# jameshensman/pyvb

Hardware: AMD Instinct MI355X
Metric: VB update iterations/sec (T=10k, D=64, N=1024 LDS); ELBO rel-err vs NumPy (higher is better)
Workload: dtype f64; 1 GPU; LDS T=10000 D=64 K=64, 1024 replicates per GPU (BASELINE configs[2]); replicates_total=1024, parallelism=replicates sharded over 1 GPU(s), collective=none (1 GPU), degraded=False

## Files before the change

### pyvb_amd/csrc/api.hip

```cpp
#include "common.h"
#include <cstdarg>
#include <cstdio>
#include <cstdlib>
#include <cstring>
#include <cmath>
#include <vector>
#include <mutex>
#include <dlfcn.h>

static thread_local char g_err[512] = "";

void pyvb_set_error(const char* fmt, ...) {
    va_list ap; va_start(ap, fmt);
    vsnprintf(g_err, sizeof(g_err), fmt, ap);
    va_end(ap);
}

int pyvb_hip_fail(hipError_t e, const char* what, const char* file, int line) {
    pyvb_set_error("HIP error %d (%s) in %s at %s:%d", (int)e, hipGetErrorString(e), what, file, line);
    return PYVB_E_HIP;
}

TimedLaunch::TimedLaunch(pyvb_lds* h_, int k_, hipStream_t s_) : h(h_), slot(-1), s(s_ ? s_ : h_->stream) {
    if (!h->timing) return;
// ... 80 lines not shown
    h->pool = (EventPair*)calloc(PYVB_EVENT_POOL, sizeof(EventPair));
    for (int i = 0; i < PYVB_EVENT_POOL; ++i) { TRYHIP(hipEventCreate(&h->pool[i].e0)); TRYHIP(hipEventCreate(&h->pool[i].e1)); }
    const size_t n = (size_t)N;
    TRY(dev_alloc(&h->Y, n * T * K));
    TRY(dev_alloc(&h->Syy, n * K));
    TRY(dev_alloc(&h->X[0], n * T * L.DP));
    TRY(dev_alloc(&h->X[1], n * T * L.DP));
    TRY(dev_alloc(&h->A_mean, n * D * D));
    TRY(dev_alloc(&h->A_var, n * D * D));
    TRY(dev_alloc(&h->C_mean, n * K * D));
    TRY(dev_alloc(&h->C_var, n * D * K));
    TRY(dev_alloc(&h->Q_a, n * D)); TRY(dev_alloc(&h->Q_b, n * D));
    TRY(dev_alloc(&h->R_a, n * K)); TRY(dev_alloc(&h->R_b, n * K));
    TRY(dev_alloc(&h->qld_A, n * D)); TRY(dev_alloc(&h->qld_C, n * D));
    TRY(dev_alloc(&h->Sigma, n * 3 * D * D)); TRY(dev_alloc(&h->Sigma_new, n * 3 * D * D));
    TRY(dev_alloc(&h->qld_x, n * 3)); TRY(dev_alloc(&h->qld_x_new, n * 3));
    TRY(dev_alloc(&h->lnd_A, n * D)); TRY(dev_alloc(&h->lnd_C, n * D));
    TRY(dev_alloc(&h->lnd_x, n * 3)); TRY(dev_alloc(&h->lnd_x_new, n * 3));
    TRY(dev_alloc(&h->gains, n * L.gains_total));
    TRY(dev_alloc(&h->scratch, g.scratch));
    TRY(dev_alloc(&h->zeros, 128));
    TRY(dev_alloc(&h->U, n * T * L.DP));
    TRY(h->mem.alloc((void**)&h->warm, n * 2 * sizeof(int)));
    TRY(dev_alloc(&h->stats, g.stats));
    TRY(dev_alloc(&h->mom, g.mom));
    TRY(dev_alloc(&h->sxx, g.sxx));
    if (g.U2) TRY(dev_alloc(&h->U2, g.U2));
    TRY(dev_alloc(&h->trash, g.trash));
    TRY(dev_alloc(&h->resQ, n * D)); TRY(dev_alloc(&h->resR, n * K));
    TRY(dev_alloc(&h->elbo, n * 6)); TRY(dev_alloc(&h->elbo_sum, 8));
    TRY(dev_alloc(&h->elbo_hist, (size_t)PYVB_ELBO_HISTORY * 8));
    TRY(h->mem.alloc((void**)&h->status, n * sizeof(int)));
    TRY(h->mem.alloc((void**)&h->active, n, 1));
    TRY(h->mem.alloc((void**)&h->counted, n, 1));
    TRY(h->mem.alloc((void**)&h->conv, n));
    TRY(h->mem.alloc((void**)&h->conv_iters, n * sizeof(int)));
    TRY(h->mem.alloc((void**)&h->conv_llb, n * sizeof(double), 0xFF));
    TRYHIP(hipHostMalloc((void**)&h->running_host, sizeof(double), hipHostMallocDefault));
    TRYHIP(hipEventCreateWithFlags(&h->ev_check, hipEventDisableTiming));
    if (ragged) {
        TRY(h->mem.alloc((void**)&h->len, n * sizeof(int)));
        TRYHIP(hipMemcpy(h->len, lengths, n * sizeof(int), hipMemcpyHostToDevice));
    }
    if (tied) {
        const Replicates& r = h->rep;
        TRY(h->mem.alloc((void**)&h->mstart, r.model_starts().size() * sizeof(int)));
        TRY(h->mem.alloc((void**)&h->first, n));
        TRYHIP(hipMemcpy(h->mstart, r.model_starts().data(), r.model_starts().size() * sizeof(int), hipMemcpyHostToDevice));
        TRYHIP(hipMemcpy(h->first, r.first_flags().data(), n, hipMemcpyHostToDevice));
    }
    h->status_host.assign(n, 0);
    h->reported.assign(n, 0);
    TRY(dev_alloc(&h->pri_block, g.priors));
    double* p = h->pri_block;
    h->pri.x0_mean = p; p += D; h->pri.x0_prec = p; p += D * D;
    h->pri.A_pm = p; p += D * D; h->pri.A_pp = p; p += D * D;
    h->pri.C_pm = p; p += K * D; h->pri.C_pp = p; p += D * K;
    h->pri.Q_a0 = p; p += D; h->pri.Q_b0 = p; p += D; h->pri.R_a0 = p; p += K; h->pri.R_b0 = p; p += K;
    h->pri.A_obs = p; p += D * D; h->pri.C_obs = p; p += K * D;
    h->pri.A_pld = p; p += D; h->pri.C_pld = p; p += D;
    h->pri.Q_w0 = p; p += D * D; h->pri.R_w0 = p; p += K * K;
    if (h->dense) {
        TRY(dev_alloc(&h->Q_w, n * D * D)); TRY(dev_alloc(&h->R_w, n * K * K));
        TRY(dev_alloc(&h->Qbar, n * D * D)); TRY(dev_alloc(&h->Rbar, n * K * K));
        TRY(dev_alloc(&h->lnd, n * 4));
        TRY(dev_alloc(&h->QA, n * D * D)); TRY(dev_alloc(&h->RC, n * K * D));
        TRY(dev_alloc(&h->trA, n * D)); TRY(dev_alloc(&h->trC, n * D));
        TRY(dev_alloc(&h->A_cov, n * D * cov_stride(D))); TRY(dev_alloc(&h->C_cov, n * D * cov_stride(K)));
        TRY(dev_alloc(&h->SyyF, n * K * K));
        TRY(dev_alloc(&h->RQ, n * D * D)); TRY(dev_alloc(&h->RR, n * K * K));
        TRY(dev_alloc(&h->SG, g.SG));
        TRY(dev_alloc(&h->ldm, n * 2 * D));
    }
    TRYHIP(hipMemset(h->pri.A_obs, 0xFF, ((size_t)D * D + (size_t)K * D) * sizeof(double)));
    h->st.T = T;
    h->st.fresh = (unsigned char*)calloc(T, 1);
    h->world = 1;
    {
        std::vector<double> nanv(n * (size_t)(D > 3 ? D : 3), NAN);
        TRYHIP(hipMemcpy(h->qld_x, nanv.data(), n * 3 * sizeof(double), hipMemcpyHostToDevice));
        TRYHIP(hipMemcpy(h->qld_A, nanv.data(), n * D * sizeof(double), hipMemcpyHostToDevice));
        TRYHIP(hipMemcpy(h->qld_C, nanv.data(), n * D * sizeof(double), hipMemcpyHostToDevice));
        TRYHIP(hipMemcpy(h->lnd_x, nanv.data(), n * 3 * sizeof(double), hipMemcpyHostToDevice));
        TRYHIP(hipMemcpy(h->lnd_A, nanv.data(), n * D * sizeof(double), hipMemcpyHostToDevice));
        TRYHIP(hipMemcpy(h->lnd_C, nanv.data(), n * D * sizeof(double), hipMemcpyHostToDevice));
    }
#undef dev_alloc
#undef TRY
#undef TRYHIP
    *out = h;
    return PYVB_OK;
}

int pyvb_lds_create(pyvb_lds** out, int device, int N, int T, int D, int K, int noise_kind) {
    return lds_create(out, device, N, T, D, K, noise_kind, nullptr, nullptr);
}
int pyvb_lds_create_lengths(pyvb_lds** out, int device, int N, int T, int D, int K, int noise_kind, const int* lengths) {
    return lds_create(out, device, N, T, D, K, noise_kind, lengths, nullptr);
}
int pyvb_lds_create_tied(pyvb_lds** out, int device, int N, int T, int D, int K, int noise_kind, const int* lengths, const int* model) {
    return lds_create(out, device, N, T, D, K, noise_kind, lengths, model);
}

int pyvb_lds_get_models(pyvb_lds* h, int* model) {
    ARGCHK(h, "handle is NULL");
    ARGCHK(model, "model is NULL");
// ... 32 lines not shown
    if (h->rep.n_active() == h->N) return PYVB_OK;
    int rc;
    if (h->st.x_park != h->st.cur && (rc = launch_carry(h, h->X[h->st.x_park], h->X[h->st.cur], (size_t)h->T * h->L.DP))) return rc;
    if (h->st.cls_parked_other) {
        if ((rc = launch_carry(h, h->Sigma_new, h->Sigma, (size_t)3 * h->D * h->D))) return rc;
        if ((rc = launch_carry(h, h->qld_x_new, h->qld_x, 3))) return rc;
        if ((rc = launch_carry(h, h->lnd_x_new, h->lnd_x, 3))) return rc;
    }
    h->st.parked_here();
    return PYVB_OK;
}

static int h2d(pyvb_lds* h, double* dst, const double* src, size_t n) { return to_device(h->stream, dst, src, n); }
static int d2h(pyvb_lds* h, double* dst, const double* src, size_t n) { return to_host(h->stream, dst, src, n); }

static void fill_padding(const pyvb_lds* h, double* a, size_t per, double value) {
    if (!h->rep.ragged() || !a) return;
    for (size_t n = 0; n < (size_t)h->N; ++n)
        for (size_t i = ((size_t)n * h->T + h->rep.length((int)n)) * per; i < (size_t)(n + 1) * h->T * per; ++i) a[i] = value;
}

static int host_lndet(const double* Ain, int D, double* out) {
    std::vector<double> A(Ain, Ain + (size_t)D * D);
    double s = 0.0;
    for (int j = 0; j < D; ++j) {
        double piv = A[j * D + j];
        for (int k = 0; k < j; ++k) piv -= A[j * D + k] * A[j * D + k];
        if (!(piv > 0.0)) return PYVB_E_LINALG;
        double d = sqrt(piv);
        A[j * D + j] = d; s += log(d);
        for (int i = j + 1; i < D; ++i) {
            double v = A[i * D + j];
            for (int k = 0; k < j; ++k) v -= A[i * D + k] * A[j * D + k];
            A[i * D + j] = v / d;
        }
    }
    *out = 2.0 * s;
    return PYVB_OK;
}

int pyvb_lds_set_priors(pyvb_lds* h, const double* x0_mean, const double* x0_prec,
                        const double* A_pm, const double* A_pp, const double* C_pm, const double* C_pp,
                        const double* Q_a0, const double* Q_b0, const double* R_a0, const double* R_b0) {
    ENTER(h);
    ARGCHK(x0_mean && x0_prec && A_pm && A_pp && C_pm && C_pp, "the priors of X_0 and of the columns are required");
    ARGCHK(h->dense || (Q_a0 && Q_b0 && R_a0 && R_b0), "the Gamma priors of Q and R are required");
    const int D = h->D, K = h->K, N = h->N;
    for (int i = 0; i < D * D; ++i) ARGCHK(A_pp[i] > 0.0, "A_prior_prec must be positive");
    for (int i = 0; i < D * K; ++i) ARGCHK(C_pp[i] > 0.0, "C_prior_prec must be positive");
    if (host_lndet(x0_prec, D, &h->pri.x0_lndet) != PYVB_OK) { pyvb_set_error("x0_prec is not positive definite"); return PYVB_E_LINALG; }
    int rc;
    if ((rc = h2d(h, h->pri.x0_mean, x0_mean, D))) return rc;
    if ((rc = h2d(h, h->pri.x0_prec, x0_prec, (size_t)D * D))) return rc;
    if ((rc = h2d(h, h->pri.A_pm, A_pm, (size_t)D * D))) return rc;
    if ((rc = h2d(h, h->pri.A_pp, A_pp, (size_t)D * D))) return rc;
    if ((rc = h2d(h, h->pri.C_pm, C_pm, (size_t)K * D))) return rc;
    if ((rc = h2d(h, h->pri.C_pp, C_pp, (size_t)D * K))) return rc;
    {
        std::vector<double> ld(2 * (size_t)D, 0.0);
        for (int i = 0; i < D; ++i) {
            for (int k = 0; k < D; ++k) ld[i] += log(A_pp[(size_t)i * D + k]);
            for (int k = 0; k < K; ++k) ld[D + i] += log(C_pp[(size_t)i * K + k]);
        }
        HIPCHK(hipMemcpyAsync(h->pri.A_pld, ld.data(), 2 * (size_t)D * sizeof(double), hipMemcpyHostToDevice, h->stream));
        HIPCHK(hipStreamSynchronize(h->stream));
    }
    if (!h->dense) {
        if ((rc = h2d(h, h->pri.Q_a0, Q_a0, D))) return rc;
        if ((rc = h2d(h, h->pri.Q_b0, Q_b0, D))) return rc;
        if ((rc = h2d(h, h->pri.R_a0, R_a0, K))) return rc;
        if ((rc = h2d(h, h->pri.R_b0, R_b0, K))) return rc;
        std::vector<double> qa((size_t)N * D), ra((size_t)N * K);
        std::vector<long> cq, cr;
        h->rep.children(cq, cr);
        for (int n = 0; n < N; ++n) {
            const long nq = cq[n], nr = cr[n];
            for (int k = 0; k < D; ++k)
                qa[(size_t)n * D + k] = (h->noise == PYVB_NOISE_GAMMA) ? Q_a0[0] + 0.5 * D * nq : Q_a0[k] + 0.5 * nq;
            for (int k = 0; k < K; ++k)
                ra[(size_t)n * K + k] = (h->noise == PYVB_NOISE_GAMMA) ? R_a0[0] + 0.5 * K * nr : R_a0[k] + 0.5 * nr;
        }
        if ((rc = h2d(h, h->Q_a, qa.data(), qa.size()))) return rc;
        if ((rc = h2d(h, h->R_a, ra.data(), ra.size()))) return rc;
        HIPCHK(hipStreamSynchronize(h->stream));
    }
    h->ard[0].on = h->ard[1].on = false;
    h->st.parameters_changed();
    return PYVB_OK;
}

static int ard_which(const pyvb_lds* h, int which, bool need_on) {
    ARGCHK(which == 0 || which == 1, "which must be 0 (A) or 1 (C)");
    if (need_on && !h->ard[which].on) {
        pyvb_set_error("the columns of %s have Constant precision parents: no hyperpriors were given (pyvb_lds_set_column_precisions)",
                       which == 0 ? "A" : "C");
        return PYVB_E_ARG;
    }
    return PYVB_OK;
}

int pyvb_lds_set_column_precisions(pyvb_lds* h, int which, const double* a0, const double* b0, const double* qb) {
    ARGCHK(h, "handle is NULL");
    int rc = ard_which(h, which, false);
    if (rc) return rc;
    if (h->dense) {
        pyvb_set_error("Gamma precision parents of the columns are served with DiagonalGamma and Gamma noise only, not with Wishart noise (k_wishart.hip)");
// ... 970 lines not shown
```

### pyvb_amd/csrc/common.h

```cpp
#pragma once
#include <cstdint>
#include "host.h"
#include "geometry.h"
#include "replicates.h"

struct pyvb_comm;
typedef double d4 __attribute__((ext_vector_type(4)));
typedef double d2 __attribute__((ext_vector_type(2)));

struct Priors {
    double *x0_mean, *x0_prec, *A_pm, *A_pp, *C_pm, *C_pp, *Q_a0, *Q_b0, *R_a0, *R_b0;
    double *A_obs, *C_obs;
    double *Q_w0, *R_w0;
    double *A_pld, *C_pld;
    double x0_lndet;
    double Q_a0_host, R_a0_host, Q_w0_lndet, R_w0_lndet;
};

struct ArdBuffers {
    bool on;
    double *a0, *b0, *qa;
    double *qb, *ex, *ld_ref, *ld_exact;
};

struct EventPair;
struct KernelTimer {
    double total_ms; int launches;
};

struct pyvb_lds {
    int device, N, T, D, K, noise;
    bool big;
    double* U2;
    Layout L;
    hipStream_t stream;
    struct EventPair* pool; int pool_used;
    double *Y, *Syy;
    double *X[2];
    double *A_mean, *A_var, *C_mean, *C_var;
    double *Q_a, *Q_b, *R_a, *R_b;
    double *qld_A, *qld_C;
    double *lnd_A, *lnd_C;
    int bound;
    Priors pri;
    double *pri_block;
    ArdBuffers ard[2];
    double *Sigma, *qld_x;
    double *Sigma_new, *qld_x_new;
    double *lnd_x, *lnd_x_new;
    double *gains;
    double *scratch;
    int *warm;
    double *zeros;
    double *trash;
    double *U;
    double *stats; int nchunk, chunk_len;
    int W;
    double *sxx;
    double *mom;
    double *resQ, *resR;
    double *elbo, *elbo_sum;
    int *status;
    Replicates rep;
    unsigned char *active;
    unsigned char *counted;
    unsigned char *conv;
    int *conv_iters;
    double *conv_llb;
    double *running_host;
    hipEvent_t ev_check;
    int *len;
    int *mstart;
    unsigned char *first;
    std::vector<int> status_host, reported;
    LdsState st;
    DeviceBuffers mem;
    bool timing; KernelTimer timers[PYVB_K_COUNT]; int timing_errors;
    pyvb_comm* comm; int rank, world;
    bool dense;
    double *Q_w, *R_w;
    double *Qbar, *Rbar;
    double *lnd;
    double *QA, *RC;
    double *trA, *trC;
    double *A_cov, *C_cov;
    double *SyyF;
    double *RQ, *RR;
    double *ldm;
    double *SG;
    bool has_missing;
    double *Yobs, *Yvar, *Yqld, *Yent;
    double *Ylnd, *YentX;
    double *Yld, *YcovS;
    hipStream_t side;
    hipEvent_t ev_params, ev_elbo;
    bool elbo_in_flight;
    double* elbo_hist; int hist_count;
};
#define PYVB_ELBO_HISTORY 4096

int launch_prep(pyvb_lds* h);
int launch_sweep(pyvb_lds* h, int direction, int src, bool read_cache, bool keep_x);
int launch_step(pyvb_lds* h, int t);
int launch_syy(pyvb_lds* h);
int launch_permute(pyvb_lds* h, const double* src, double* dst, int to_internal);
int launch_carry(pyvb_lds* h, const double* src, double* dst, size_t per);
int launch_stats(pyvb_lds* h, bool with_sxx);
int launch_moments(pyvb_lds* h, bool sxx_from_sweep);
int launch_observe(pyvb_lds* h);
int launch_tie(pyvb_lds* h, double* buf, size_t per);
int launch_cols(pyvb_lds* h, int which, int c0, int c1, int fuse = 0);
int launch_resid(pyvb_lds* h, int which);
int launch_ard(pyvb_lds* h, int which, bool derive);
int launch_noise(pyvb_lds* h, int which);
int launch_elbo(pyvb_lds* h, hipStream_t stream = nullptr);
int launch_elbo_sum(pyvb_lds* h, double* out = nullptr, hipStream_t stream = nullptr);
int launch_converge(pyvb_lds* h, double tol, bool first, hipStream_t stream);
int launch_prep_big(pyvb_lds* h);
int big_prepare_kernels();
int launch_sweep_big(pyvb_lds* h, int direction, int src, bool cached);
int launch_step_big(pyvb_lds* h, int t);
int launch_stats_big(pyvb_lds* h);
int launch_cols_big(pyvb_lds* h, int which, int c0, int c1, int fuse);
int launch_wexpect(pyvb_lds* h);
int launch_dense_pre(pyvb_lds* h);
int launch_cols_dense(pyvb_lds* h, int which, int c0, int c1);
int launch_wresid(pyvb_lds* h, int which, int update, bool use_sg);
int launch_syy_full(pyvb_lds* h);
int launch_elbo_dense(pyvb_lds* h, hipStream_t stream = nullptr);
int launch_colvar_to_cov(pyvb_lds* h);
int launch_cov_to_colvar(pyvb_lds* h);
int launch_cov_observe(pyvb_lds* h);
int launch_cov_convert(pyvb_lds* h, int which, double* dense, int n0, int count, int to_packed);
int launch_wexpect_big(pyvb_lds* h);
int launch_dense_pre_big(pyvb_lds* h);
int launch_cols_dense_big(pyvb_lds* h, int which, int c0, int c1);
int launch_wresid_big(pyvb_lds* h, int which, int update, bool use_sg);
int launch_syy_full_big(pyvb_lds* h);
int launch_missing_init(pyvb_lds* h, const double* Yq0, const double* Yrowvar0);
int launch_impute(pyvb_lds* h);
int launch_syy_missing(pyvb_lds* h);
int launch_impute_dense(pyvb_lds* h);
int launch_missing_ent_dense(pyvb_lds* h, int diag_cov);

struct pyvb_comm {
    void* nccl;
    pyvb_host_allreduce_fn fn; void* user;
    double* host; size_t cap;
};
int pyvb_comm_create(pyvb_comm** comm, const char id[128], int rank, int world);
int pyvb_comm_create_host(pyvb_comm** comm, pyvb_host_allreduce_fn fn, void* user);
void pyvb_comm_free(pyvb_comm* comm);
int pyvb_allreduce_f64(pyvb_comm* comm, double* buf, size_t count, hipStream_t stream);

// ... 9 lines not shown
```

### pyvb_amd/csrc/k_prep.hip

```cpp
#include "common.h"
#include "gj.h"

struct PrepArgs {
    const double *A_mean, *A_var, *C_mean, *C_var, *Q_a, *Q_b, *R_a, *R_b, *x0_mean, *x0_prec;
    double *Sigma, *qld, *lnd, *gains, *scratch;
    const double *Qbar, *QA, *RC, *trA, *trC;
    int *warm, *status;
    const unsigned char* active;
    int N, T, D, K;
    Layout L;
};

#define PREP_THREADS 256
#define MFMA(a, b, c) __builtin_amdgcn_mfma_f64_16x16x4f64((a), (b), (c), 0, 0, 0)

template <int MT, int NT, int KS, class FA, class FB, class FS>
__device__ __forceinline__ void mm(int wave, int lane, FA a_at, FB b_at, FS store) {
    const int r = lane & 15, q = lane >> 4;
    for (int m = wave; m < MT; m += 4) {
        d4 acc[NT];
#pragma unroll
        for (int n = 0; n < NT; ++n) acc[n] = d4{0, 0, 0, 0};
#pragma unroll 4
        for (int s = 0; s < KS; ++s) {
            const double av = a_at(16 * m + r, 4 * s + q);
#pragma unroll
            for (int n = 0; n < NT; ++n) acc[n] = MFMA(av, b_at(4 * s + q, 16 * n + r), acc[n]);
        }
#pragma unroll
        for (int n = 0; n < NT; ++n)
#pragma unroll
            for (int e = 0; e < 4; ++e) store(16 * m + 4 * e + q, 16 * n + r, acc[n][e]);
    }
}

template <int NT, int KS, class FA, class FB>
__device__ __forceinline__ void mm_acc(int m, int lane, FA a_at, FB b_at, d4 (&acc)[NT]) {
    const int r = lane & 15, q = lane >> 4;
#pragma unroll
    for (int n = 0; n < NT; ++n) acc[n] = d4{0, 0, 0, 0};
#pragma unroll 4
    for (int s = 0; s < KS; ++s) {
        const double av = a_at(16 * m + r, 4 * s + q);
#pragma unroll
        for (int n = 0; n < NT; ++n) acc[n] = MFMA(av, b_at(4 * s + q, 16 * n + r), acc[n]);
    }
}
template <int NT, class FS>
__device__ __forceinline__ void mm_out(int m, int lane, const d4 (&acc)[NT], FS store) {
    const int r = lane & 15, q = lane >> 4;
#pragma unroll
    for (int n = 0; n < NT; ++n)
#pragma unroll
        for (int e = 0; e < 4; ++e) store(16 * m + 4 * e + q, 16 * n + r, acc[n][e]);
}

__device__ __forceinline__ double inf_norm(const double* A, int LD, int D, int tid, double* red) {
// ... 151 lines not shown
    __syncthreads();
    gj_inverse<3>(sig, D, tid, gjbuf, gjbuf + 3 * 2 * GJ_BUF);
    if (tid < 64) {
#pragma unroll
        for (int c = 0; c < 3; ++c) {
            double lp = 0.0;
            if (tid < D) {
                const double piv = gjbuf[3 * 2 * GJ_BUF + c * 64 + tid];
                if (!(piv > 0.0)) atomicOr(a.status + n, PYVB_FAIL_STATES);
                lp = log(piv);
            }
#pragma unroll
            for (int o = 32; o > 0; o >>= 1) lp += __shfl_xor(lp, o, 64);
            if (tid == 0) { a.qld[(size_t)n * 3 + c] = 0.5 / (0.5 * lp); a.lnd[(size_t)n * 3 + c] = -lp; }
        }
    }
    if ((D & 3) == 0) {
#pragma unroll
        for (int c = 0; c < 3; ++c)
#pragma unroll
            for (int ra = 0; ra < 4; ++ra) {
                const int i = 4 * ta + ra, j0 = 4 * tb;
                if (i < D && j0 < D)
                    *reinterpret_cast<d4*>(a.Sigma + ((size_t)n * 3 + c) * D * D + (size_t)i * D + j0) = d4{sig[c][4 * ra], sig[c][4 * ra + 1], sig[c][4 * ra + 2], sig[c][4 * ra + 3]};
            }
    } else {
#pragma unroll
    for (int c = 0; c < 3; ++c)
#pragma unroll
        for (int ra = 0; ra < 4; ++ra)
#pragma unroll
            for (int cb = 0; cb < 4; ++cb) {
                const int i = 4 * ta + ra, j = 4 * tb + cb;
                if (i < D && j < D) a.Sigma[((size_t)n * 3 + c) * D * D + i * D + j] = sig[c][4 * ra + cb];
            }
    }

#pragma unroll
    for (int ra = 0; ra < 4; ++ra) {
        const int i = 4 * ta + ra, j0 = 4 * tb;
        if (i < DP && j0 < DP) {
            d4 s0, s2;
#pragma unroll
            for (int cb = 0; cb < 4; ++cb) {
                const bool in = i < D && j0 + cb < D;
                s0[cb] = in ? sig[0][4 * ra + cb] : 0.0;
                s2[cb] = in ? sig[2][4 * ra + cb] : 0.0;
            }
            *reinterpret_cast<d4*>(g + L.oS0 + (size_t)i * DP + j0) = s0;
            *reinterpret_cast<d4*>(g + L.oS2 + (size_t)i * DP + j0) = s2;
        }
    }
    if (tid < 64) { g[L.oqr + tid] = qbar[tid]; g[L.oqr + 64 + tid] = rbar[tid]; }
    if (tid < DP) {
        double s = 0.0;
        if (tid < D) for (int j = 0; j < D; ++j) s += a.x0_prec[tid * D + j] * a.x0_mean[j];
        g[L.ow0 + tid] = s;
    }
#pragma unroll
    for (int ra = 0; ra < 4; ++ra)
#pragma unroll
        for (int cb = 0; cb < 4; ++cb) {
            const int i = 4 * ta + ra, j = 4 * tb + cb;
            if (i < D && j < D) P[i * LD + j] = sig[1][4 * ra + cb];
        }
    __syncthreads();
    if constexpr (STAGE) {
        constexpr int KP = 16 * KT;
        for (int idx = tid; idx < DP * DP; idx += PREP_THREADS) W[(idx / DP) * LD + idx % DP] = qbar[idx / DP] * A_at(idx / DP, idx % DP);
        __syncthreads();
        d4 facc[DT], acc[DT], gacc[KT];
        if (wave < DT) {
            mm_acc<DT, DS>(wave, lane, [&](int i, int k) { return P[i * LD + k]; }, [&](int k, int j) { return W[k * LD + j]; }, facc);
            mm_out<DT>(wave, lane, facc, [&](int i, int j, double v) { if (i < D && j < D) g[L.oFn + pos_nat(i, j, DS)] = v; });
            mm_acc<DT, DS>(wave, lane, [&](int i, int k) { return P[i * LD + k]; }, [&](int k, int j) { return W[j * LD + k]; }, acc);
            mm_out<DT>(wave, lane, acc, [&](int i, int j, double v) { if (i < D && j < D) g[L.oBn + pos_nat(i, j, DS)] = v; });
        }
        __syncthreads();
        for (int idx = tid; idx < KP * DP; idx += PREP_THREADS) W[(idx / DP) * LD + idx % DP] = rbar[idx / DP] * C_at(idx / DP, idx % DP);
        __syncthreads();
        if (wave < DT) {
            mm_acc<KT, DS>(wave, lane, [&](int i, int k) { return P[i * LD + k]; }, [&](int k, int l) { return W[l * LD + k]; }, gacc);
            mm_out<KT>(wave, lane, gacc, [&](int i, int l, double v) { if (i < D && l < K) g[L.oGp + pos_perm(i, l, KS)] = v; });
        }
        __syncthreads();
        if (wave < DT) mm_out<DT>(wave, lane, facc, [&](int i, int j, double v) { W[i * LD + j] = (i < D && j < D) ? v : 0.0; });
    } else
    {
        mm<DT, DT, DS>(wave, lane,
                       [&](int i, int k) { return P[i * LD + k]; },
                       [&](int k, int j) { if constexpr (DENSE) return QA_at(k, j); else return qbar[k] * A_at(k, j); },
                       [&](int i, int j, double v) {
                           if (i < D && j < D) { g[L.oFn + pos_nat(i, j, DS)] = v; W[i * LD + j] = v; }
                       });
        mm<DT, DT, DS>(wave, lane,
                       [&](int i, int k) { return P[i * LD + k]; },
                       [&](int k, int j) { if constexpr (DENSE) return QA_at(j, k); else return A_at(j, k) * qbar[j]; },
                       [&](int i, int j, double v) {
                           if (i < D && j < D) g[L.oBn + pos_nat(i, j, DS)] = v;
                       });
        mm<DT, KT, DS>(wave, lane,
                       [&](int i, int k) { return P[i * LD + k]; },
                       [&](int k, int l) { if constexpr (DENSE) return RC_at(l, k); else return C_at(l, k) * rbar[l]; },
                       [&](int i, int l, double v) {
                           if (i < D && l < K) g[L.oGp + pos_perm(i, l, KS)] = v;
                       });
    }
    __syncthreads();

    int J = warmup_length<DT>(W, P, LD, D, tid, rowp);
    if (tid == 0) a.warm[n * 2 + 0] = J;
    __syncthreads();
    for (int idx = tid; idx < DP * LD; idx += PREP_THREADS) {
        const int i = idx / LD, j = idx % LD;
        W[idx] = (i < D && j < D) ? g[L.oBn + pos_nat(j, i, DS)] : 0.0;
    }
    __syncthreads();
    J = warmup_length<DT>(W, P, LD, D, tid, rowp);
    if (tid == 0) a.warm[n * 2 + 1] = J;
}

template <int DT, int KT>
static void launch_prep_t(pyvb_lds* h, const PrepArgs& a) {
    if (h->dense) hipLaunchKernelGGL((k_prep<DT, KT, true>), dim3(h->N), dim3(PREP_THREADS), 0, h->stream, a);
    else hipLaunchKernelGGL((k_prep<DT, KT, false>), dim3(h->N), dim3(PREP_THREADS), 0, h->stream, a);
}

int launch_prep(pyvb_lds* h) {
    if (h->big) return launch_prep_big(h);
    PrepArgs a;
    a.A_mean = h->A_mean; a.A_var = h->A_var; a.C_mean = h->C_mean; a.C_var = h->C_var;
    a.Q_a = h->Q_a; a.Q_b = h->Q_b; a.R_a = h->R_a; a.R_b = h->R_b;
    a.x0_mean = h->pri.x0_mean; a.x0_prec = h->pri.x0_prec;
    a.Sigma = h->Sigma_new; a.qld = h->qld_x_new; a.lnd = h->lnd_x_new; a.gains = h->gains; a.scratch = h->scratch;
    a.warm = h->warm; a.status = h->status; a.active = h->active;
    a.Qbar = h->Qbar; a.QA = h->QA; a.RC = h->RC; a.trA = h->trA; a.trC = h->trC;
    a.N = h->N; a.T = h->T; a.D = h->D; a.K = h->K; a.L = h->L;
    {
        TimedLaunch tl(h, PYVB_K_PREP);
        switch (h->L.DT * 10 + h->L.KT) {
            case 11: launch_prep_t<1, 1>(h, a); break;
            case 12: launch_prep_t<1, 2>(h, a); break;
            case 14: launch_prep_t<1, 4>(h, a); break;
            case 21: launch_prep_t<2, 1>(h, a); break;
            case 22: launch_prep_t<2, 2>(h, a); break;
            case 24: launch_prep_t<2, 4>(h, a); break;
            case 41: launch_prep_t<4, 1>(h, a); break;
            case 42: launch_prep_t<4, 2>(h, a); break;
            case 44: launch_prep_t<4, 4>(h, a); break;
            default: pyvb_set_error("unsupported tile shape"); return PYVB_E_ARG;
        }
    }
    HIPCHK(hipGetLastError());
    return PYVB_OK;
}
```

### pyvb_amd/csrc/k_sweep.hip

```cpp
#include "common.h"

struct SweepArgs {
    const double* Xold; double* Xnew; const double* Y; const double* gains; const int* warm;
    const double *A_mean, *C_mean;
    const double *QA, *RC;
    double* trash;
    double* U;
    double* Sxx;
    int N, T, D, K, dir;
    int W;
    const unsigned char* active;
    const int* len;
    int keep_x;
    Layout L;
};

#define MFMA(a, b, c) __builtin_amdgcn_mfma_f64_16x16x4f64((a), (b), (c), 0, 0, 0)

template <class NB>
__device__ __forceinline__ double boundary_update(bool first, const double* g, const Layout& L, const double* Am, const double* Cm,
                                                  int D, int K, int lane, NB nb, const double* y, double* vs,
                                                  const double* QA = nullptr, const double* RC = nullptr) {
    const double* qb = g + L.oqr;
    const double* rb = qb + 64;
    double v = 0.0;
    if (QA) {
        if (lane < D) {
            if (first) {
                v = g[L.ow0 + lane];
                for (int i = 0; i < D; ++i) v += QA[(size_t)i * D + lane] * nb(i);
            } else {
                for (int j = 0; j < D; ++j) v += QA[(size_t)lane * D + j] * nb(j);
            }
            for (int k = 0; k < K; ++k) v += RC[(size_t)k * D + lane] * y[k];
        }
    } else if (lane < D) {
        if (first) {
            v = g[L.ow0 + lane];
            for (int i = 0; i < D; ++i) v += Am[(size_t)i * D + lane] * (qb[i] * nb(i));
        } else {
            double s = 0.0;
            for (int j = 0; j < D; ++j) s += Am[(size_t)lane * D + j] * nb(j);
            v = qb[lane] * s;
        }
        for (int k = 0; k < K; ++k) v += Cm[(size_t)k * D + lane] * (rb[k] * y[k]);
    }
    vs[lane] = v;
    __syncthreads();
    const double* S = g + (first ? L.oS0 : L.oS2);
    double s = 0.0;
    if (lane < D)
        for (int j = 0; j < D; ++j) s += S[(size_t)j * L.DP + lane] * vs[j];
    __syncthreads();
    return s;
}

template <int DT, int KT, bool FULL, int MODE, bool SPLIT>
__global__ void __launch_bounds__(64) k_sweep(SweepArgs a) {
    constexpr int DS = 4 * DT, KS = 4 * KT, DP = 16 * DT;
    __shared__ double gl[MODE == 2 ? DP * 17 : DT * KS * 64];
    __shared__ double xs[64];
    __shared__ double vs[64];
    const int n = blockIdx.x, w = SPLIT ? blockIdx.y : 0, lane = threadIdx.x, c = lane & 15, q = lane >> 4;
    if (!a.active[n]) return;
    const int T = a.T, D = a.D, K = a.K;
    const int TL = a.len ? a.len[n] : T;
    const bool fwd = (a.dir == 0);
    const int sgn = fwd ? 1 : -1;
    const Layout& L = a.L;
    const double* g = a.gains + (size_t)n * L.gains_total;
    const double* Xo = a.Xold + (size_t)n * T * DP;
    double* Xn = a.Xnew + (size_t)n * T * DP;
    const double* Yn = a.Y + (size_t)n * T * K;

    double rn[DT][DS], ip[DT][DS];
    {
        const double* Rn = g + (fwd ? L.oFn : L.oBn);
        const double* Ip = g + (fwd ? L.oBn : L.oFn);
#pragma unroll
        for (int m = 0; m < DT; ++m)
#pragma unroll
            for (int s = 0; s < DS; ++s) {
                rn[m][s] = Rn[(m * DS + s) * 64 + lane];
                ip[m][s] = (MODE == 2) ? 0.0 : Ip[(m * DS + s) * 64 + lane];
            }
        if constexpr (MODE != 2) {
            const double* Gp = g + L.oGp;
            for (int i = 0; i < DT * KS; ++i) gl[i * 64 + lane] = Gp[i * 64 + lane];
        }
    }

    const int Tint = TL - 2;
    const int Lw = SPLIT ? split_part_len(T, a.W) : Tint;
    const int ow = SPLIT ? w * Lw : 0;
    const int Tw = (Tint - ow < Lw) ? Tint - ow : Lw;
    const int J = a.warm[n * 2 + a.dir];

    const int t_first = fwd ? 0 : TL - 1, t_last = fwd ? TL - 1 : 0;
    const double* Am = a.A_mean + (size_t)n * D * D;
    const double* Cm = a.C_mean + (size_t)n * K * D;
    const double* QAm = a.QA ? a.QA + (size_t)n * D * D : nullptr;
    const double* RCm = a.RC ? a.RC + (size_t)n * K * D : nullptr;
    if (!SPLIT || ow <= J) {
        const double* xo = Xo + (size_t)(t_first + sgn) * DP;
        const double s = boundary_update(fwd, g, L, Am, Cm, D, K, lane, [&](int j) { return xo[xpos(j)]; },
                                         Yn + (size_t)t_first * K, vs, QAm, RCm);
        if (w == 0 && lane < DP) Xn[(size_t)t_first * DP + xpos(lane)] = (lane < D) ? s : 0.0;
        xs[lane] = (lane < D) ? s : 0.0;
    }
    __builtin_amdgcn_fence(__ATOMIC_RELEASE, "workgroup");
    __builtin_amdgcn_s_barrier();
    __builtin_amdgcn_fence(__ATOMIC_ACQUIRE, "workgroup");

    if (Tw > 0) {
        const int Lseg = (Tw + 15) >> 4;
        const int cL = c * Lseg;
        const int before = ow + cL;
        const int jc = -(J < before ? J : before);
        const int jstart = -((J < ow + 15 * Lseg) ? J : ow + 15 * Lseg);
        d4 x[DT];
#pragma unroll
        for (int m = 0; m < DT; ++m)
#pragma unroll
            for (int r = 0; r < 4; ++r) x[m][r] = (jc == -before) ? xs[16 * m + 4 * r + q] : 0.0;

        const int tbase = fwd ? (1 + before) : (TL - 2 - before);
        const int tsafe = fwd ? 1 : TL - 2;
        auto active = [&](int j) { int tt = cL + j; return j >= jc && j < Lseg && tt < Tw; };
        d2 yv[KS / 2];
        d4 mo[DT];
        auto load_y = [&](int j, d2* dst) {
            const double* p = Yn + (size_t)(active(j) ? tbase + sgn * j : tsafe) * K;
#pragma unroll
            for (int i = 0; i < KS / 2; ++i) {
                const int d0 = 8 * i + 2 * q;
                if constexpr (FULL) {
                    dst[i] = *reinterpret_cast<const d2*>(p + d0);
                } else {
                    dst[i][0] = p[d0 < K ? d0 : K - 1];
                    dst[i][1] = p[d0 + 1 < K ? d0 + 1 : K - 1];
                }
            }
        };
        auto load_o = [&](int j, d4* dst) {
            const double* p = Xo + (size_t)((active(j) ? tbase + sgn * j : tsafe) + sgn) * DP;
#pragma unroll
            for (int m = 0; m < DT; ++m) dst[m] = *reinterpret_cast<const d4*>(p + (m * 4 + q) * 4);
        };
        auto store_x = [&](double* out) {
#pragma unroll
            for (int m = 0; m < DT; ++m) *reinterpret_cast<d4*>(out + (m * 4 + q) * 4) = x[m];
        };
        double* const trash = a.trash + (size_t)n * 256;
        double* out_pending = trash;
        double* const Un = a.U + (size_t)n * T * DP;
        auto u_row = [&](int j) { return (active(j) && j >= 0) ? Un + (size_t)(tbase + sgn * j) * DP : trash; };
        auto load_u = [&](int j, d4* dst) {
            const double* p = Un + (size_t)(active(j) ? tbase + sgn * j : tsafe) * DP;
#pragma unroll
// ... 89 lines not shown
        } else {
        load_y(jstart, yv);
        store_x(trash);
        if constexpr (MODE == 1) store_x(trash + 64);
        load_o(jstart, mo);
        for (int j = jstart; j < Lseg; ++j) {
            d4 acc[DT];
            {
#pragma unroll
                for (int m = 0; m < DT; ++m) acc[m] = d4{0.0, 0.0, 0.0, 0.0};
                int goff = lane;
                asm volatile("" : "+v"(goff));
#pragma unroll
                for (int s = 0; s < KS; ++s)
#pragma unroll
                    for (int m = 0; m < DT; ++m) acc[m] = MFMA(gl[(m * KS + s) * 64 + goff], yv[s >> 1][s & 1], acc[m]);
                __builtin_amdgcn_sched_barrier(0);
                load_y(j + 1, yv);
                store_x(out_pending);
                __builtin_amdgcn_sched_barrier(0);
            }
            mul_resident(acc, rn, x);
            {
                if constexpr (MODE == 1) {
                    __builtin_amdgcn_sched_barrier(0);
                    double* ur = u_row(j);
#pragma unroll
                    for (int m = 0; m < DT; ++m) *reinterpret_cast<d4*>(ur + (m * 4 + q) * 4) = acc[m];
                    __builtin_amdgcn_sched_barrier(0);
                }
                mul_resident(acc, ip, mo);
                __builtin_amdgcn_sched_barrier(0);
                load_o(j + 1, mo);
                __builtin_amdgcn_sched_barrier(0);
            }
            finish_step(j, acc);
        }
        store_x(out_pending);
        }
        const int clast = (Tw - 1) / Lseg;
        __builtin_amdgcn_s_barrier();
        if (c == clast) {
#pragma unroll
            for (int m = 0; m < DT; ++m)
#pragma unroll
                for (int r = 0; r < 4; ++r) xs[16 * m + 4 * r + q] = x[m][r];
        }
        __builtin_amdgcn_fence(__ATOMIC_RELEASE, "workgroup");
        __builtin_amdgcn_s_barrier();
        __builtin_amdgcn_fence(__ATOMIC_ACQUIRE, "workgroup");
    }

    if (!SPLIT || w == ((Tint > 0) ? (Tint - 1) / Lw : 0)) {
        const double s = boundary_update(!fwd, g, L, Am, Cm, D, K, lane, [&](int j) { return xs[j]; },
                                         Yn + (size_t)t_last * K, vs, QAm, RCm);
        if (lane < DP) Xn[(size_t)t_last * DP + xpos(lane)] = (lane < D) ? s : 0.0;
    }
}

struct StepArgs {
    double* X; const double* Y; const double* gains; const double *A_mean, *C_mean, *QA, *RC;
    const unsigned char* active;
    const int* len;
    int N, T, D, K, t;
    Layout L;
};

__global__ void __launch_bounds__(64) k_step(StepArgs a) {
    const int n = blockIdx.x, lane = threadIdx.x;
    if (!a.active[n]) return;
    const int T = a.T, D = a.D, K = a.K, t = a.t, DP = a.L.DP;
    const int TL = a.len ? a.len[n] : T;
    if (t >= TL) return;
    const Layout& L = a.L;
    const double* g = a.gains + (size_t)n * L.gains_total;
    double* X = a.X + (size_t)n * T * DP;
    const double* y = a.Y + ((size_t)n * T + t) * K;
    const int cls = (t == 0) ? 0 : (t == TL - 1 ? 2 : 1);
    const int row = lane % DP;
    if (cls != 1) {
        __shared__ double vs[64];
        const double* nbr = X + (size_t)(cls == 0 ? 1 : TL - 2) * DP;
        const double s = boundary_update(cls == 0, g, L, a.A_mean + (size_t)n * D * D, a.C_mean + (size_t)n * K * D, D, K, lane,
                                         [&](int j) { return nbr[xpos(j)]; }, y, vs,
                                         a.QA ? a.QA + (size_t)n * D * D : nullptr, a.RC ? a.RC + (size_t)n * K * D : nullptr);
        if (lane < DP) X[(size_t)t * DP + xpos(lane)] = (lane < D) ? s : 0.0;
        return;
    }
    const int DS = L.DS, KS = L.KS;
    double s = 0.0;
    for (int j = 0; j < D; ++j) s += g[L.oFn + pos_nat(row, j, DS)] * X[(size_t)(t - 1) * DP + xpos(j)];
    for (int j = 0; j < D; ++j) s += g[L.oBn + pos_nat(row, j, DS)] * X[(size_t)(t + 1) * DP + xpos(j)];
    for (int k = 0; k < K; ++k) s += g[L.oGp + pos_perm(row, k, KS)] * y[k];
    if (lane < DP) X[(size_t)t * DP + xpos(lane)] = (lane < D) ? s : 0.0;
}

template <int DT, int KT>
static int launch_sweep_t(pyvb_lds* h, const SweepArgs& a, bool read_cache) {
    const bool full = h->D == 16 * DT && h->K == 16 * KT;
    const int mode = a.dir == PYVB_FORWARD ? 1 : (read_cache ? 2 : 0);
#define PYVB_SWEEP_CASE(F, M) do { if (h->W > 1) hipLaunchKernelGGL((k_sweep<DT, KT, F, M, true>), dim3(h->N, h->W), dim3(64), 0, h->stream, a); \
                                   else hipLaunchKernelGGL((k_sweep<DT, KT, F, M, false>), dim3(h->N), dim3(64), 0, h->stream, a); } while (0)
    if (full) { if (mode == 1) PYVB_SWEEP_CASE(true, 1); else if (mode == 2) PYVB_SWEEP_CASE(true, 2); else PYVB_SWEEP_CASE(true, 0); }
    else { if (mode == 1) PYVB_SWEEP_CASE(false, 1); else if (mode == 2) PYVB_SWEEP_CASE(false, 2); else PYVB_SWEEP_CASE(false, 0); }
#undef PYVB_SWEEP_CASE
    return PYVB_OK;
}

int launch_sweep(pyvb_lds* h, int direction, int src, bool read_cache, bool keep_x) {
    if (h->big) return launch_sweep_big(h, direction, src, read_cache);
    SweepArgs a;
    a.keep_x = (keep_x || direction != PYVB_FORWARD) ? 1 : 0;
    a.W = h->W;
    a.Xold = h->X[src]; a.Xnew = h->X[1 - src]; a.Y = h->Y; a.gains = h->gains; a.warm = h->warm;
    a.trash = h->trash; a.U = h->U; a.Sxx = h->sxx; a.A_mean = h->A_mean; a.C_mean = h->C_mean;
    a.QA = h->dense ? h->QA : nullptr; a.RC = h->dense ? h->RC : nullptr;
    a.N = h->N; a.T = h->T; a.D = h->D; a.K = h->K; a.dir = direction; a.L = h->L; a.active = h->active; a.len = h->len;
    {
        TimedLaunch tl(h, direction == PYVB_FORWARD ? PYVB_K_SWEEP_FWD : PYVB_K_SWEEP_BWD);
        switch (h->L.DT * 10 + h->L.KT) {
            case 11: launch_sweep_t<1, 1>(h, a, read_cache); break;
            case 12: launch_sweep_t<1, 2>(h, a, read_cache); break;
            case 14: launch_sweep_t<1, 4>(h, a, read_cache); break;
            case 21: launch_sweep_t<2, 1>(h, a, read_cache); break;
            case 22: launch_sweep_t<2, 2>(h, a, read_cache); break;
            case 24: launch_sweep_t<2, 4>(h, a, read_cache); break;
            case 41: launch_sweep_t<4, 1>(h, a, read_cache); break;
            case 42: launch_sweep_t<4, 2>(h, a, read_cache); break;
            case 44: launch_sweep_t<4, 4>(h, a, read_cache); break;
            default: pyvb_set_error("unsupported tile shape"); return PYVB_E_ARG;
        }
    }
    HIPCHK(hipGetLastError());
    return PYVB_OK;
}

struct PermArgs { const double* src; double* dst; size_t rows; int D, DP, to_internal; };
__global__ void __launch_bounds__(256) k_permute(PermArgs a) {
// ... 45 lines not shown
```

Baseline: 89.04 VB iterations/s per 1024 replicates (whole job).

## Restructure sweep boundary update into blocked unrolled chains and hoist x0 prior product

Rewrites the boundary update at the sweep endpoints. The neighbour state, the observation row and the intermediate vector are now staged in LDS, and each dot product runs as compile-time-unrolled blocks of 16 loads followed by FMAs, replacing serial loops that reread through a lambda and interleaved loads with FMAs. This targets the fixed per-launch latency of each sweep. Separately, the prior product x0_prec*x0_mean is computed once by a new one-block kernel when priors are set, not per replicate in every prep launch. The cost is extra LDS arrays, more barriers and clamped redundant loads for padded lanes. A profiling script is added to separate the per-launch cost from the per-step cost of the sweeps.

```diff
diff --git a/profiles/sweep_fixed_cost.py b/profiles/sweep_fixed_cost.py
--- /dev/null
+++ b/profiles/sweep_fixed_cost.py
@@ -0,0 +1,69 @@
+import argparse
+import os
+import sys
+
+REPO = os.path.dirname(os.path.dirname(os.path.abspath(__file__)))
+sys.path.insert(0, REPO)
+
+D, N = 64, 1024
+LENGTHS = (2502, 5002, 10002)
+
+
+def fit(x, y):
+    import numpy as np
+    x, y = np.asarray(x, dtype=float), np.asarray(y, dtype=float)
+    b, a = np.polyfit(x, y, 1)
+    return a, b, float(np.abs(a + b * x - y).max())
+
+
+def main():
+    ap = argparse.ArgumentParser()
+    ap.add_argument("--steps", type=int, default=6)
+    ap.add_argument("--warmup", type=int, default=3)
+    ap.add_argument("--label", default="")
+    ap.add_argument("--out")
+    args = ap.parse_args()
+    lines = []
+
+    def say(text):
+        print(text, flush=True)
+        lines.append(text)
+
+    from bench import make_inputs
+    from pyvb_amd.lds import LDSBatch
+
+    Yfull, st_full, pri = make_inputs(max(LENGTHS), D, D, N, seed=20240)
+    pts = {"sweep_fwd": [], "sweep_bwd": []}
+    steps_mean, steps_max = {"sweep_fwd": [], "sweep_bwd": []}, {"sweep_fwd": [], "sweep_bwd": []}
+    for T in LENGTHS:
+        st0 = {k: (v[:, :T] if k == "X" else v) for k, v in st_full.items()}
+        b = LDSBatch.from_problem(Yfull[:, :T], st0, pri)
+        assert b.get_time_split() == 1
+        b.iterate(args.warmup); b.sync()
+        b.timing(True)
+        b.iterate(args.steps); b.sync()
+        kt = b.kernel_times()
+        b.timing(False)
+        w = b.get_warmup()
+        b.close()
+        lseg = (T - 2 + 15) // 16
+        for col, nm in enumerate(("sweep_fwd", "sweep_bwd")):
+            ms, cnt = kt[nm]
+            assert cnt == args.steps, (nm, cnt)
+            pts[nm].append(ms / cnt)
+            steps_mean[nm].append(lseg + float(w[:, col].mean()))
+            steps_max[nm].append(lseg + int(w[:, col].max()))
+            say("%sT %6d  %-9s %8.4f ms per launch   loop steps %4d + J (mean %.1f, max %d)" % (
+                args.label, T, nm, ms / cnt, lseg, w[:, col].mean(), w[:, col].max()))
+    for nm in ("sweep_fwd", "sweep_bwd"):
+        a, bb, res = fit(steps_mean[nm], pts[nm])
+        a2, b2, res2 = fit(steps_max[nm], pts[nm])
+        say("%s%-9s a = %7.4f ms per launch, b = %.5f ms per step (largest residual %.4f ms);  with the largest J: a = %7.4f, b = %.5f (%.4f)" % (
+            args.label, nm, a, bb, res, a2, b2, res2))
+    if args.out:
+        with open(args.out, "a") as f:
+            f.write("\n".join(lines) + "\n")
+
+
+if __name__ == "__main__":
+    main()
diff --git a/pyvb_amd/csrc/api.hip b/pyvb_amd/csrc/api.hip
--- a/pyvb_amd/csrc/api.hip
+++ b/pyvb_amd/csrc/api.hip
@@ -156,6 +156,7 @@
     h->status_host.assign(n, 0);
     h->reported.assign(n, 0);
     TRY(dev_alloc(&h->pri_block, g.priors));
+    TRY(dev_alloc(&h->w0, L.DP));
     double* p = h->pri_block;
     h->pri.x0_mean = p; p += D; h->pri.x0_prec = p; p += D * D;
     h->pri.A_pm = p; p += D * D; h->pri.A_pp = p; p += D * D;
@@ -294,6 +295,7 @@
     int rc;
     if ((rc = h2d(h, h->pri.x0_mean, x0_mean, D))) return rc;
     if ((rc = h2d(h, h->pri.x0_prec, x0_prec, (size_t)D * D))) return rc;
+    if (!h->big && (rc = launch_w0(h))) return rc;
     if ((rc = h2d(h, h->pri.A_pm, A_pm, (size_t)D * D))) return rc;
     if ((rc = h2d(h, h->pri.A_pp, A_pp, (size_t)D * D))) return rc;
     if ((rc = h2d(h, h->pri.C_pm, C_pm, (size_t)K * D))) return rc;
diff --git a/pyvb_amd/csrc/common.h b/pyvb_amd/csrc/common.h
--- a/pyvb_amd/csrc/common.h
+++ b/pyvb_amd/csrc/common.h
@@ -44,6 +44,7 @@
     int bound;
     Priors pri;
     double *pri_block;
+    double *w0;
     ArdBuffers ard[2];
     double *Sigma, *qld_x;
     double *Sigma_new, *qld_x_new;
@@ -100,6 +101,7 @@
 #define PYVB_ELBO_HISTORY 4096
 
 int launch_prep(pyvb_lds* h);
+int launch_w0(pyvb_lds* h);
 int launch_sweep(pyvb_lds* h, int direction, int src, bool read_cache, bool keep_x);
 int launch_step(pyvb_lds* h, int t);
 int launch_syy(pyvb_lds* h);
diff --git a/pyvb_amd/csrc/k_prep.hip b/pyvb_amd/csrc/k_prep.hip
--- a/pyvb_amd/csrc/k_prep.hip
+++ b/pyvb_amd/csrc/k_prep.hip
@@ -2,7 +2,8 @@
 #include "gj.h"
 
 struct PrepArgs {
-    const double *A_mean, *A_var, *C_mean, *C_var, *Q_a, *Q_b, *R_a, *R_b, *x0_mean, *x0_prec;
+    const double *A_mean, *A_var, *C_mean, *C_var, *Q_a, *Q_b, *R_a, *R_b, *x0_prec;
+    const double* w0;
     double *Sigma, *qld, *lnd, *gains, *scratch;
     const double *Qbar, *QA, *RC, *trA, *trC;
     int *warm, *status;
@@ -260,11 +261,7 @@
         }
     }
     if (tid < 64) { g[L.oqr + tid] = qbar[tid]; g[L.oqr + 64 + tid] = rbar[tid]; }
-    if (tid < DP) {
-        double s = 0.0;
-        if (tid < D) for (int j = 0; j < D; ++j) s += a.x0_prec[tid * D + j] * a.x0_mean[j];
-        g[L.ow0 + tid] = s;
-    }
+    if (tid < DP) g[L.ow0 + tid] = a.w0[tid];
 #pragma unroll
     for (int ra = 0; ra < 4; ++ra)
 #pragma unroll
@@ -328,6 +325,22 @@
     if (tid == 0) a.warm[n * 2 + 1] = J;
 }
 
+struct W0Args { const double *x0_mean, *x0_prec; double* w0; int D, DP; };
+__global__ void __launch_bounds__(128) k_w0(W0Args a) {
+    const int tid = threadIdx.x, D = a.D;
+    if (tid >= a.DP) return;
+    double s = 0.0;
+    if (tid < D) for (int j = 0; j < D; ++j) s += a.x0_prec[tid * D + j] * a.x0_mean[j];
+    a.w0[tid] = s;
+}
+
+int launch_w0(pyvb_lds* h) {
+    W0Args a; a.x0_mean = h->pri.x0_mean; a.x0_prec = h->pri.x0_prec; a.w0 = h->w0; a.D = h->D; a.DP = h->L.DP;
+    hipLaunchKernelGGL(k_w0, dim3(1), dim3(128), 0, h->stream, a);
+    HIPCHK(hipGetLastError());
+    return PYVB_OK;
+}
+
 template <int DT, int KT>
 static void launch_prep_t(pyvb_lds* h, const PrepArgs& a) {
     if (h->dense) hipLaunchKernelGGL((k_prep<DT, KT, true>), dim3(h->N), dim3(PREP_THREADS), 0, h->stream, a);
@@ -339,7 +352,7 @@
     PrepArgs a;
     a.A_mean = h->A_mean; a.A_var = h->A_var; a.C_mean = h->C_mean; a.C_var = h->C_var;
     a.Q_a = h->Q_a; a.Q_b = h->Q_b; a.R_a = h->R_a; a.R_b = h->R_b;
-    a.x0_mean = h->pri.x0_mean; a.x0_prec = h->pri.x0_prec;
+    a.x0_prec = h->pri.x0_prec; a.w0 = h->w0;
     a.Sigma = h->Sigma_new; a.qld = h->qld_x_new; a.lnd = h->lnd_x_new; a.gains = h->gains; a.scratch = h->scratch;
     a.warm = h->warm; a.status = h->status; a.active = h->active;
     a.Qbar = h->Qbar; a.QA = h->QA; a.RC = h->RC; a.trA = h->trA; a.trC = h->trC;
diff --git a/pyvb_amd/csrc/k_sweep.hip b/pyvb_amd/csrc/k_sweep.hip
--- a/pyvb_amd/csrc/k_sweep.hip
+++ b/pyvb_amd/csrc/k_sweep.hip
@@ -17,50 +17,48 @@
 
 #define MFMA(a, b, c) __builtin_amdgcn_mfma_f64_16x16x4f64((a), (b), (c), 0, 0, 0)
 
-template <class NB>
+constexpr int BOUNDARY_BLOCK = 16;
+
+template <int NP>
+__device__ __forceinline__ double boundary_chain(double v, const double* M, size_t stride, size_t off, int n, const double* u) {
+#pragma unroll
+    for (int b = 0; b < NP; b += BOUNDARY_BLOCK) {
+        if (b >= n) break;
+        double m[BOUNDARY_BLOCK];
+#pragma unroll
+        for (int e = 0; e < BOUNDARY_BLOCK; ++e) m[e] = M[(size_t)(b + e < n ? b + e : n - 1) * stride + off];
+#pragma unroll
+        for (int e = 0; e < BOUNDARY_BLOCK; ++e) v += (b + e < n ? m[e] : 0.0) * u[b + e];
+    }
+    return v;
+}
+
+template <int DP, int KP>
 __device__ __forceinline__ double boundary_update(bool first, const double* g, const Layout& L, const double* Am, const double* Cm,
-                                                  int D, int K, int lane, NB nb, const double* y, double* vs,
+                                                  int D, int K, int lane, double xn, const double* y, double* ux, double* uy, double* vs,
                                                   const double* QA = nullptr, const double* RC = nullptr) {
-    const double* qb = g + L.oqr;
-    const double* rb = qb + 64;
-    double v = 0.0;
-    if (QA) {
-        if (lane < D) {
-            if (first) {
-                v = g[L.ow0 + lane];
-                for (int i = 0; i < D; ++i) v += QA[(size_t)i * D + lane] * nb(i);
-            } else {
-                for (int j = 0; j < D; ++j) v += QA[(size_t)lane * D + j] * nb(j);
-            }
-            for (int k = 0; k < K; ++k) v += RC[(size_t)k * D + lane] * y[k];
-        }
-    } else if (lane < D) {
-        if (first) {
-            v = g[L.ow0 + lane];
-            for (int i = 0; i < D; ++i) v += Am[(size_t)i * D + lane] * (qb[i] * nb(i));
-        } else {
-            double s = 0.0;
-            for (int j = 0; j < D; ++j) s += Am[(size_t)lane * D + j] * nb(j);
-            v = qb[lane] * s;
-        }
-        for (int k = 0; k < K; ++k) v += Cm[(size_t)k * D + lane] * (rb[k] * y[k]);
-    }
-    vs[lane] = v;
+    const bool dense = QA != nullptr;
+    const int lc = lane < D ? lane : D - 1, kc = lane < K ? lane : K - 1;
+    const double qb = g[L.oqr + lc], rb = g[L.oqr + 64 + kc], yk = y[kc], w0 = g[L.ow0 + lc];
+    ux[lane] = lane < D ? ((first && !dense) ? qb * xn : xn) : 0.0;
+    uy[lane] = lane < K ? (dense ? yk : rb * yk) : 0.0;
     __syncthreads();
-    const double* S = g + (first ? L.oS0 : L.oS2);
-    double s = 0.0;
-    if (lane < D)
-        for (int j = 0; j < D; ++j) s += S[(size_t)j * L.DP + lane] * vs[j];
+    double v = boundary_chain<DP>(first ? w0 : 0.0, dense ? QA : Am, first ? D : 1, (size_t)lc * (first ? 1 : D), D, ux);
+    if (!first && !dense) v = qb * v;
+    v = boundary_chain<KP>(v, dense ? RC : Cm, D, lc, K, uy);
+    vs[lane] = lane < D ? v : 0.0;
     __syncthreads();
-    return s;
+    const double s = boundary_chain<DP>(0.0, g + (first ? L.oS0 : L.oS2), L.DP, lc, D, vs);
+    __syncthreads();
+    return lane < D ? s : 0.0;
 }
 
 template <int DT, int KT, bool FULL, int MODE, bool SPLIT>
 __global__ void __launch_bounds__(64) k_sweep(SweepArgs a) {
-    constexpr int DS = 4 * DT, KS = 4 * KT, DP = 16 * DT;
+    constexpr int DS = 4 * DT, KS = 4 * KT, DP = 16 * DT, KP = 16 * KT;
     __shared__ double gl[MODE == 2 ? DP * 17 : DT * KS * 64];
     __shared__ double xs[64];
-    __shared__ double vs[64];
+    __shared__ double vs[64], ux[64], uy[64];
     const int n = blockIdx.x, w = SPLIT ? blockIdx.y : 0, lane = threadIdx.x, c = lane & 15, q = lane >> 4;
     if (!a.active[n]) return;
     const int T = a.T, D = a.D, K = a.K;
@@ -103,8 +101,8 @@
     const double* RCm = a.RC ? a.RC + (size_t)n * K * D : nullptr;
     if (!SPLIT || ow <= J) {
         const double* xo = Xo + (size_t)(t_first + sgn) * DP;
-        const double s = boundary_update(fwd, g, L, Am, Cm, D, K, lane, [&](int j) { return xo[xpos(j)]; },
-                                         Yn + (size_t)t_first * K, vs, QAm, RCm);
+        const double s = boundary_update<DP, KP>(fwd, g, L, Am, Cm, D, K, lane, xo[xpos(lane < D ? lane : D - 1)],
+                                                 Yn + (size_t)t_first * K, ux, uy, vs, QAm, RCm);
         if (w == 0 && lane < DP) Xn[(size_t)t_first * DP + xpos(lane)] = (lane < D) ? s : 0.0;
         xs[lane] = (lane < D) ? s : 0.0;
     }
@@ -300,8 +298,8 @@
     }
 
     if (!SPLIT || w == ((Tint > 0) ? (Tint - 1) / Lw : 0)) {
-        const double s = boundary_update(!fwd, g, L, Am, Cm, D, K, lane, [&](int j) { return xs[j]; },
-                                         Yn + (size_t)t_last * K, vs, QAm, RCm);
+        const double s = boundary_update<DP, KP>(!fwd, g, L, Am, Cm, D, K, lane, xs[lane],
+                                                 Yn + (size_t)t_last * K, ux, uy, vs, QAm, RCm);
         if (lane < DP) Xn[(size_t)t_last * DP + xpos(lane)] = (lane < D) ? s : 0.0;
     }
 }
@@ -327,11 +325,11 @@
     const int cls = (t == 0) ? 0 : (t == TL - 1 ? 2 : 1);
     const int row = lane % DP;
     if (cls != 1) {
-        __shared__ double vs[64];
+        __shared__ double vs[64], ux[64], uy[64];
         const double* nbr = X + (size_t)(cls == 0 ? 1 : TL - 2) * DP;
-        const double s = boundary_update(cls == 0, g, L, a.A_mean + (size_t)n * D * D, a.C_mean + (size_t)n * K * D, D, K, lane,
-                                         [&](int j) { return nbr[xpos(j)]; }, y, vs,
-                                         a.QA ? a.QA + (size_t)n * D * D : nullptr, a.RC ? a.RC + (size_t)n * K * D : nullptr);
+        const double s = boundary_update<64, 64>(cls == 0, g, L, a.A_mean + (size_t)n * D * D, a.C_mean + (size_t)n * K * D, D, K, lane,
+                                                 nbr[xpos(lane < D ? lane : D - 1)], y, ux, uy, vs,
+                                                 a.QA ? a.QA + (size_t)n * D * D : nullptr, a.RC ? a.RC + (size_t)n * K * D : nullptr);
         if (lane < DP) X[(size_t)t * DP + xpos(lane)] = (lane < D) ? s : 0.0;
         return;
     }
```

Result: faster. 90.27 VB iterations/s per 1024 replicates (whole job) (median of 6 runs) (+1.4%).
